# LukasHedegaard/continual-skeletons

Hardware: AMD Instinct MI355X
Metric: clips/sec (ST-GCN clip forward, NTU-60 shape; CoST-GCN online step reported under costgcn_online) (higher is better)
Workload: dtype f32

## Files before the change

### continual-skeletons_amd/blocks.py

```python
import math

import numpy as np
import torch
import torch.nn as nn
from torch.nn.modules.batchnorm import _BatchNorm
from torch.nn.modules.conv import _ConvNd

from . import fold, native


def init_weights(module_, bs=1):
    if isinstance(module_, _ConvNd):
        nn.init.constant_(module_.bias, 0)
        if bs == 1:
            nn.init.kaiming_normal_(module_.weight, mode="fan_out")
        else:
            nn.init.normal_(module_.weight, 0, math.sqrt(2.0 / (module_.weight.numel() * bs)))
    elif isinstance(module_, _BatchNorm):
        nn.init.constant_(module_.weight, bs)
        nn.init.constant_(module_.bias, 0)
    elif isinstance(module_, nn.Linear):
        nn.init.normal_(module_.weight, 0, math.sqrt(2.0 / bs))


# ... 201 lines not shown
        if self.clip_split_k <= 1 or type(self) is not GraphConvolution or self.in_channels < 16:
            return 1
        return max(1, min(self.clip_split_k, -(-self.in_channels // 8)))

    def stage(self, x, y, n_seg, frames, x_strides, y_strides, ksplit=1, partial=None):
        ops = self._packed_ops(x.device)
        if ksplit > 1:
            rc = native.lib().csk_gcn_stage_splitk_f32(
                native.ptr(x), native.ptr(y), native.ptr(ops["w"]), native.ptr(ops["bias"]), native.ptr(ops["ell_src"]),
                native.ptr(ops["ell_val"]), native.ptr(ops["ell_cnt_host"]), ops["ell_w"], n_seg, ops["c_in"], ops["c_out"], frames,
                ops["V"], x_strides[0], x_strides[1], y_strides[0], y_strides[1], ops["res_mode"], ksplit, native.ptr(partial),
                native.stream_of(x))
            native.check(rc, "csk_gcn_stage_splitk_f32")
            return
        gcn_stage(x, y, ops, n_seg=n_seg, frames=frames, x_strides=x_strides, y_strides=y_strides)


def gcn_stage(x, y, ops, n_seg, frames, x_strides, y_strides, adj_seg_stride=0, adj_per_frame=0):
    rc = native.lib().csk_gcn_stage_f32(
        native.ptr(x), native.ptr(y), native.ptr(ops["w"]), native.ptr(ops["bias"]),
        native.ptr(ops["ell_src"]), native.ptr(ops["ell_val"]), native.ptr(ops["ell_cnt_host"]),
        ops["ell_w"], adj_seg_stride, adj_per_frame, n_seg, ops["c_in"], ops["c_out"], frames, ops["V"],
        x_strides[0], x_strides[1], y_strides[0], y_strides[1], ops["res_mode"], native.stream_of(x),
    )
    native.check(rc, "csk_gcn_stage_f32")


class TemporalConvolution(_Folded):

    def __init__(self, in_channels, out_channels, kernel_size=9, stride=1, padding=4):
        super().__init__()
        self.padding = padding
        self.stride = stride
        self.kernel_size = kernel_size
        self.t_conv = nn.Conv2d(in_channels, out_channels, kernel_size=(kernel_size, 1), padding=(padding, 0),
                                stride=(stride, 1))
        self.bn = nn.BatchNorm2d(out_channels)
        init_weights(self.t_conv, bs=1)
        init_weights(self.bn, bs=1)

    def _fold(self):
        f = fold.fold_temporal_conv(self.state_dict())
        f["bias"] = fold.pad_vec(f["bias"])
        return f

    def forward(self, x):
        self._require_eval()
        _check_input(x, self.t_conv.in_channels, "TemporalConvolution input")
        ops = self._packed_ops(x.device)
        return tcn_stage(x, ops["w"], ops["bias"], ops["c_out"], ops["k"], self.stride, self.padding, relu=False)


def tcn_stage(y, w, bias, c_out, k, stride, pad, relu=True, res_mode=0, x_res=None, w_res=None, res_off=0, out=None,
              split=False, ksplit=1, scratch=None, w_wino=None):
    n, c, t_in, v = y.shape
    if t_in + 2 * pad < k:
        raise RuntimeError(f"temporal extent {t_in} (+2*{pad}) shorter than kernel {k}")
    t_out = (t_in + 2 * pad - k) // stride + 1
    if out is None:
        out = torch.empty((n, c_out, t_out, v), device=y.device, dtype=torch.float32)
    elif tuple(out.shape) != (n, c_out, t_out, v) or not out.is_contiguous() or out.dtype != torch.float32 or out.device != y.device:
        raise RuntimeError(f"out must be a contiguous float32 {(n, c_out, t_out, v)} tensor on {y.device}")
    c_res, t_res = (x_res.shape[1], x_res.shape[2]) if x_res is not None else (0, 0)
    if ksplit > 1 and not split:
        if scratch is None:
            raise RuntimeError("tcn_stage: ksplit > 1 needs the owning module's SplitScratch")
        part = scratch.get(y.device, ksplit * n * c_out * t_out * v)
        rc = native.lib().csk_tcn_stage_splitk_f32(
            native.ptr(y), native.ptr(w), native.ptr(x_res), native.ptr(w_res), native.ptr(bias), native.ptr(out),
            n, c, c_out, t_in, v, k, stride, pad, res_mode, c_res, t_res, res_off, int(relu), ksplit, native.ptr(part),
            native.stream_of(y))
        native.check(rc, "csk_tcn_stage_splitk_f32")
        return out
    if w_wino is not None and not split:
        rc = native.lib().csk_tcn_stage_wino_f32(
            native.ptr(y), native.ptr(w), native.ptr(x_res), native.ptr(w_res), native.ptr(bias), native.ptr(out),
            n, c, c_out, t_in, v, k, stride, pad, res_mode, c_res, t_res, res_off, int(relu), native.ptr(w_wino),
            native.stream_of(y))
        native.check(rc, "csk_tcn_stage_wino_f32")
        return out
    fn = native.lib().csk_tcn_stage_bf16x3 if split else native.lib().csk_tcn_stage_f32
    rc = fn(native.ptr(y), native.ptr(w), native.ptr(x_res), native.ptr(w_res), native.ptr(bias), native.ptr(out),
            n, c, c_out, t_in, v, k, stride, pad, res_mode, c_res, t_res, res_off, int(relu), native.stream_of(y))
    native.check(rc, "csk_tcn_stage_bf16x3" if split else "csk_tcn_stage_f32")
    return out


class SpatioTemporalBlock(_Folded):

    def __init__(self, in_channels, out_channels, A, stride=1, residual=True, temporal_kernel_size=9,
                 temporal_padding=-1, GraphConv=GraphConvolution, TempConv=TemporalConvolution):
        super().__init__()
        equal_padding = int((temporal_kernel_size - 1) / 2)
        if temporal_padding < 0:
            temporal_padding = equal_padding
            self.residual_shrink = None
        else:
            assert temporal_padding <= equal_padding
            self.residual_shrink = equal_padding - temporal_padding
        self.stride = stride
        self.gcn = GraphConv(in_channels, out_channels, A)
        self.tcn = TempConv(out_channels, out_channels, stride=stride, kernel_size=temporal_kernel_size,
                            padding=temporal_padding)
        self.relu = nn.ReLU()
        if not residual:
            self.residual = zero
        elif (in_channels == out_channels) and (stride == 1):
            self.residual = unity
        else:
            self.residual = TempConv(in_channels, out_channels, kernel_size=1, stride=stride, padding=0)
        self._native_tail = isinstance(self.tcn, TemporalConvolution) and (
            self.residual in (zero, unity) or isinstance(self.residual, TemporalConvolution)
        )

    precision = "f32"
    clip_split_k = 0
    clip_split_max_seq = CLIP_SPLIT_MAX_SEQUENCES

    def _watched(self):
        return [m for m in (self.tcn, self.residual) if isinstance(m, nn.Module)]

    def _fold(self):
        sd = self.state_dict()
        return fold.fold_block_tail(sd, "", has_conv_residual=isinstance(self.residual, TemporalConvolution),
                                    split=self.precision == "bf16x3", stride=self.stride)

    def forward(self, x, out=None):
        self._require_eval()
        native.require_device_f32(x, "SpatioTemporalBlock input")
        if self._few_channels_fusable(x):
            return self._forward_few_channels(x, out)
        y = self.gcn(x)
        if not self._native_tail:
            z = self.tcn(y)
            r = self.residual(x[:, :, self.residual_shrink:-self.residual_shrink] if self.residual_shrink else x)
            return self.relu(z + r)
        ops = self._packed_ops(x.device)
        shrink = self.residual_shrink or 0
        if self.residual is zero:
            mode, xr = 0, None
        elif self.residual is unity:
            mode, xr = 1, x
        else:
            mode, xr = 2, x
        if self.precision == "bf16x3":
            return tcn_stage(y, ops["w_split"], ops["bias"], ops["c_out"], ops["k"], self.stride, self.tcn.padding, relu=True,
                             res_mode=mode, x_res=xr, w_res=ops["w_res_split"], res_off=shrink, out=out, split=True)
        ks = max(1, min(self.clip_split_k, -(-ops["c"] // 8))) if (self.clip_split_k > 1 and ops["k"] == 9 and y.shape[0] <= self.clip_split_max_seq) else 1
        return tcn_stage(y, ops["w"], ops["bias"], ops["c_out"], ops["k"], self.stride, self.tcn.padding, relu=True,
                         res_mode=mode, x_res=xr, w_res=ops["w_res"], res_off=shrink, out=out, ksplit=ks,
                         scratch=_scratch_of(self) if ks > 1 else None, w_wino=ops["w_wino"] if ks == 1 else None)


def _few_channels_fusable(self, x) -> bool:
    if not self.fuse_few_channels or type(self.gcn) is not GraphConvolution or not self._native_tail:
        return False
    if self.gcn.in_channels > 4 or self.residual is not zero or self.stride != 1 or self.precision != "f32" or self.residual_shrink:
        return False
    if x.dim() != 4 or x.shape[3] not in (18, 25) or self.gcn.precision != "f32":
        return False
    if self.clip_split_k > 1 and x.shape[0] <= self.clip_split_max_seq:
        return False
    g, t = self.gcn._packed_ops(x.device), self._packed_ops(x.device)
    return (t["k"] == 9 and self.tcn.padding == 4 and g["res_mode"] == 2 and g["c_out"] % 8 == 0 and g["V"] == x.shape[3]
            and max(int(v) for v in g["ell_cnt_host"][:2]) <= 1 and int(g["ell_cnt_host"][2]) <= 4)


def _forward_few_channels(self, x, out=None):
    _check_input(x, self.gcn.in_channels, "SpatioTemporalBlock input")
    g, t = self.gcn._packed_ops(x.device), self._packed_ops(x.device)
    n, c, tt, v = x.shape
    if out is None:
        out = torch.empty((n, t["c_out"], tt, v), device=x.device, dtype=torch.float32)
    rc = native.lib().csk_block_few_channels_f32(
        native.ptr(x.contiguous()), native.ptr(g["w"]), native.ptr(g["bias"]), native.ptr(g["ell_src"]), native.ptr(g["ell_val"]),
        native.ptr(g["ell_cnt_host"]), g["ell_w"], native.ptr(t["w"]), native.ptr(t["bias"]), native.ptr(out), n, c, g["c_out"],
        t["c_out"], tt, v, self.tcn.padding, native.stream_of(x))
    native.check(rc, "csk_block_few_channels_f32")
    return out


SpatioTemporalBlock.fuse_few_channels = False
SpatioTemporalBlock._few_channels_fusable = _few_channels_fusable
SpatioTemporalBlock._forward_few_channels = _forward_few_channels


def tcn_step_launch(*args):
    native.check(native.lib().csk_tcn_step_f32(*args), "csk_tcn_step_f32")
```

### continual-skeletons_amd/csrc/tcn_wino.hip

```cpp
#include "mfma_core.h"
#include "tcn_params.h"

namespace {

constexpr int WMT = 64;
constexpr int WNT = 128;
constexpr int WTAPS = 12;

template <int VT>
constexpr int wino_ldb() { return ((2 * ((WNT + VT - 2) / VT) + 10) * VT + 3) / 4 * 4; }

struct WStage12x64 {
    unsigned goff0, loff0, gstride;
    f32x4 v[6];
    __device__ __forceinline__ void setup(int Cpad, int Mpad, int tid) {
        goff0 = (unsigned)(((tid >> 7) * Cpad + ((tid >> 4) & 7)) * Mpad + (tid & 15) * 4);
        loff0 = (unsigned)(tid * 4);
        gstride = (unsigned)(2 * Cpad * Mpad);
    }
    __device__ __forceinline__ void issue_slot(int u, const float *__restrict__ chunk_base) {
        v[u] = *reinterpret_cast<const f32x4 *>(chunk_base + (size_t)u * gstride + goff0);
    }
    __device__ __forceinline__ void issue(const float *__restrict__ chunk_base) {
#pragma unroll
        for (int u = 0; u < 6; ++u) issue_slot(u, chunk_base);
    }
    __device__ __forceinline__ void commit(float *__restrict__ Wl) const {
#pragma unroll
        for (int u = 0; u < 6; ++u) *reinterpret_cast<f32x4 *>(Wl + u * (NTHREADS * 4) + loff0) = v[u];
    }
};

template <int VT, int G>
__device__ __forceinline__ void wino_group(const float *__restrict__ Wl, const float *__restrict__ Bl, int off, int l31, int kh,
                                           f32x16 (&acc)[4][2]) {
    constexpr int LDB = wino_ldb<VT>();
    const float *br = Bl + kh * LDB + off + 3 * G * VT;
    const float *wr = Wl + 4 * G * (KC * WMT) + kh * WMT + l31;
#pragma unroll
    for (int s = 0; s < KC / 2; ++s) {
        const float d0 = br[2 * s * LDB], d1 = br[2 * s * LDB + VT], d2 = br[2 * s * LDB + 2 * VT], d3 = br[2 * s * LDB + 3 * VT];
        const float b[4] = {d0 - d2, d1 + d2, d2 - d1, d1 - d3};
#pragma unroll
        for (int i = 0; i < 4; ++i) {
            const float a0 = wr[i * (KC * WMT) + 2 * s * WMT], a1 = wr[i * (KC * WMT) + 2 * s * WMT + 32];
            acc[i][0] = __builtin_amdgcn_mfma_f32_32x32x2f32(a0, b[i], acc[i][0], 0, 0, 0);
            acc[i][1] = __builtin_amdgcn_mfma_f32_32x32x2f32(a1, b[i], acc[i][1], 0, 0, 0);
        }
    }
}

}

template <int VT>
__global__ __launch_bounds__(NTHREADS, 2) void tcn_stage_wino_kernel(const TcnParams p) {
    constexpr int LDB = wino_ldb<VT>();
    constexpr int NJ = (LDB + 63) / 64;
    extern __shared__ __attribute__((aligned(16))) float smem[];
    float *Wl = smem;
    float *Bl = smem + WTAPS * KC * WMT;

    const int tid = threadIdx.x, lane = tid & 63, wave = __builtin_amdgcn_readfirstlane(tid >> 6);
    const int l31 = lane & 31, kh = lane >> 5;
    const unsigned wid = xcd_contiguous_id(blockIdx.x, gridDim.x);
    const int m0 = (int)(wid % p.mtiles) * WMT, q0 = (int)((wid / p.mtiles) % p.qtiles) * WNT;
    const int seg = (int)(wid / (p.mtiles * p.qtiles));
    const int T = p.Tout, TV = T * VT, QP = p.nt;
    const int qend = min(q0 + WNT, QP);
    const int ja = div_magic(q0, p.vmagic), jb = div_magic(qend - 1, p.vmagic);

    const int qc = min(q0 + wave * 32 + l31, qend - 1);
    const int jc = div_magic(qc, p.vmagic), vc = qc - jc * VT;
    const int off = 2 * (jc - ja) * VT + vc;

    f32x16 acc[4][2];
#pragma unroll
    for (int i = 0; i < 4; ++i)
#pragma unroll
        for (int mi = 0; mi < 2; ++mi)
#pragma unroll
            for (int g = 0; g < 16; ++g) acc[i][mi][g] = 0.f;

    {
        const int fa = 2 * ja - 4;
        const int span = (2 * (jb - ja) + 10) * VT;
        const int64_t cs = (int64_t)TV;
        const float *seg_base = p.y + (int64_t)seg * p.C * cs;
        const float *wbase = p.w + m0;
        WStage12x64 ws;
        ws.setup(p.Cpad, p.Mpad, tid);
        auto kloop = [&](auto &bx) {
            ws.issue(wbase);
            bx.issue(seg_base, p.C, cs, 0, wave);
            for (int c0 = 0; c0 + KC < p.Cpad; c0 += KC) {
                __syncthreads();
                ws.commit(Wl);
                bx.commit(Bl, LDB, wave);
                __syncthreads();
                const float *wnext = wbase + (size_t)(c0 + KC) * p.Mpad;
                const int cn = c0 + KC;
                ws.issue_slot(0, wnext);
                ws.issue_slot(1, wnext);
                bx.template issue_third<0>(seg_base, p.C, cs, cn, wave);
                __builtin_amdgcn_s_setprio(1);
                wino_group<VT, 0>(Wl, Bl, off, l31, kh, acc);
                __builtin_amdgcn_s_setprio(0);
                ws.issue_slot(2, wnext);
                ws.issue_slot(3, wnext);
                bx.template issue_third<1>(seg_base, p.C, cs, cn, wave);
                __builtin_amdgcn_s_setprio(1);
                wino_group<VT, 1>(Wl, Bl, off, l31, kh, acc);
                __builtin_amdgcn_s_setprio(0);
                ws.issue_slot(4, wnext);
                ws.issue_slot(5, wnext);
                bx.template issue_third<2>(seg_base, p.C, cs, cn, wave);
                __builtin_amdgcn_s_setprio(1);
                wino_group<VT, 2>(Wl, Bl, off, l31, kh, acc);
                __builtin_amdgcn_s_setprio(0);
            }
            __syncthreads();
            ws.commit(Wl);
            bx.commit(Bl, LDB, wave);
            __syncthreads();
            wino_group<VT, 0>(Wl, Bl, off, l31, kh, acc);
            wino_group<VT, 1>(Wl, Bl, off, l31, kh, acc);
            wino_group<VT, 2>(Wl, Bl, off, l31, kh, acc);
        };
        const bool interior = fa >= 0 && fa * VT + 4 * ((span + 3) / 4) <= TV;
        if (interior) {
            BStage4<(NJ + 3) / 4> b4;
            b4.setup(fa * VT, span, lane);
            kloop(b4);
        } else {
            BStage<NJ> bs;
            bs.setup(fa * VT, span, TV, lane);
            kloop(bs);
        }
    }

    const bool qv = q0 + wave * 32 + l31 < qend;
    const bool odd_ok = 2 * jc + 1 < T;
    const unsigned p0 = (unsigned)(2 * jc * VT + vc);
    const unsigned b0 = 4u * (4u * (unsigned)kh * (unsigned)TV + p0);
    const unsigned b1 = odd_ok ? b0 + 4u * VT : b0;
    const unsigned kh16 = 16u * (unsigned)kh;
    const float *rseg = p.xres + (int64_t)seg * p.Cout * TV;
    float *oseg = p.out + (int64_t)seg * p.Cout * TV;
#pragma unroll
    for (int mi = 0; mi < 2; ++mi) {
        const int rb = m0 + mi * 32;
        float o0[16], o1[16];
#pragma unroll
        for (int g = 0; g < 16; ++g) {
            const int row = rb + (g & 3) + 8 * (g >> 2);
            const float *rrow = rseg + (int64_t)row * TV;
            const float bias = ld_lane(p.bias + row, kh16);
            const float m1 = acc[1][mi][g], m2 = acc[2][mi][g];
            float v0 = acc[0][mi][g] + m1 + m2 + bias + ld_lane(rrow, b0);
            float v1 = m1 - m2 - acc[3][mi][g] + bias + ld_lane(rrow, b1);
            if (p.relu) { v0 = relu_nan(v0); v1 = relu_nan(v1); }
            o0[g] = v0;
            o1[g] = v1;
        }
        if (qv) {
#pragma unroll
            for (int g = 0; g < 16; ++g) {
                float *orow = oseg + (int64_t)(rb + (g & 3) + 8 * (g >> 2)) * TV;
                st_lane(orow, b0, o0[g]);
                if (odd_ok) st_lane(orow, b1, o1[g]);
            }
        }
    }
}

static int tcn_stage_wino_launch(const float *y, const float *w_wino, const float *x_res, const float *bias, float *out, int n_seg,
                                 int c, int c_out, int t_in, int V, int k, int stride, int pad, int res_mode, int c_res, int t_res,
                                 int res_off, int relu, void *stream) {
    if (!w_wino || !y || !x_res || !bias || !out) return -2;
    if (k != 9 || stride != 1 || pad != 4 || res_mode != CSK_RES_IDENTITY || res_off != 0) return -2;
    if ((V != 25 && V != 18) || c_out % WMT != 0 || c_res != c_out || t_res != t_in || c < 1 || n_seg < 1 || t_in < 1) return -2;
    if ((int64_t)t_in * V >= (1 << 26)) return -2;
    if (csk_diag_flag("CSK_TCN_WINO")) return -2;
    const int qp = (t_in + 1) / 2 * V;
    const int qtiles = (qp + WNT - 1) / WNT, mtiles = c_out / WMT;
    if ((int64_t)qtiles * mtiles * n_seg >= (1ll << 31)) return -2;
    TcnParams p = {};
    p.y = y; p.w = w_wino; p.xres = x_res; p.wres = nullptr; p.bias = bias; p.out = out;
    p.C = c; p.Cpad = round_up(c, CSK_CPAD); p.Cout = c_out; p.Mpad = round_up(c_out, CSK_MT);
    p.Tin = t_in; p.Tout = t_in; p.V = V; p.K = k; p.stride = 1; p.pad = pad;
    p.res_mode = res_mode; p.Cres = c_res; p.CresPad = round_up(c_res, CSK_CPAD); p.Tres = t_res; p.res_off = 0; p.relu = relu;
    p.vmagic = vmagic_of(V); p.mtiles = (unsigned)mtiles; p.qtiles = (unsigned)qtiles; p.nt = qp;
    void (*kern)(TcnParams) = V == 25 ? tcn_stage_wino_kernel<25> : tcn_stage_wino_kernel<18>;
    const int ldb = V == 25 ? wino_ldb<25>() : wino_ldb<18>();
    p.ldb = ldb;
    const size_t lds = (size_t)(WTAPS * KC * WMT + KC * ldb) * sizeof(float);
    if (const int e = csk_ensure_lds((const void *)kern, lds)) return e;
    hipLaunchKernelGGL(kern, dim3((unsigned)(qtiles * mtiles * n_seg)), dim3(NTHREADS), lds, (hipStream_t)stream, p);
    return (int)hipGetLastError();
}

extern "C" int csk_tcn_stage_wino_f32(const float *y, const float *w, const float *x_res, const float *w_res, const float *bias,
                                      float *out, int n_seg, int c, int c_out, int t_in, int V, int k, int stride, int pad,
                                      int res_mode, int c_res, int t_res, int res_off, int relu, const float *w_wino, void *stream) {
    const int rc = tcn_stage_wino_launch(y, w_wino, x_res, bias, out, n_seg, c, c_out, t_in, V, k, stride, pad, res_mode, c_res,
                                         t_res, res_off, relu, stream);
    if (rc != -2) return rc;
    return csk_tcn_stage_f32(y, w, x_res, w_res, bias, out, n_seg, c, c_out, t_in, V, k, stride, pad, res_mode, c_res, t_res,
                             res_off, relu, stream);
}
```

### continual-skeletons_amd/fold.py

```python
from typing import Dict, Optional, Tuple

import numpy as np
import torch

KC = 16
MT = 64
BN_EPS = 1e-5


def _ceil_to(a: int, b: int) -> int:
    return (a + b - 1) // b * b


def bn_affine(weight, bias, mean, var, eps=BN_EPS) -> Tuple[torch.Tensor, torch.Tensor]:
    s = weight.double() / torch.sqrt(var.double() + eps)
    return s, bias.double() - mean.double() * s


def pack_conv_weight(weight: torch.Tensor, scale: torch.Tensor) -> torch.Tensor:
    co, ci, k, _ = weight.shape
    w = weight.double()[:, :, :, 0] * scale[:, None, None]
    out = torch.zeros((k, _ceil_to(ci, KC), _ceil_to(co, MT)), dtype=torch.float64)
    out[:, :ci, :co] = w.permute(2, 1, 0)
    return out.float().contiguous()


WINO_G = ((1.0, 0.0, 0.0), (0.5, 0.5, 0.5), (0.5, -0.5, 0.5), (0.0, 0.0, 1.0))


def pack_conv_weight_wino(weight: torch.Tensor, scale: torch.Tensor) -> torch.Tensor:
    if weight.dim() == 4:
        weight = weight[:, :, :, 0]
    co, ci, k = weight.shape
    if k != 9:
        raise ValueError(f"the Winograd image is built for the 9 x 1 temporal conv, got k = {k}")
    w = weight.double() * scale[:, None, None]
    g = torch.tensor(WINO_G, dtype=torch.float64)
    u = torch.einsum("ir,ocgr->gico", g, w.view(co, ci, 3, 3)).reshape(12, ci, co)
    out = torch.zeros((12, _ceil_to(ci, KC), _ceil_to(co, MT)), dtype=torch.float64)
    out[:, :ci, :co] = u
    return out.float().contiguous()


SPLIT_KS = 16


def split3_bf16(w32: torch.Tensor):
    h = w32.to(torch.bfloat16)
    r1 = w32 - h.float()
    m = r1.to(torch.bfloat16)
    l = (r1 - m.float()).to(torch.bfloat16)
    return h, m, l


def pack_conv_weight_split(weight: torch.Tensor, scale: torch.Tensor, stride: int = 1) -> torch.Tensor:
    if weight.dim() == 4:
        weight = weight[:, :, :, 0]
    co, ci, k = weight.shape
    if k not in (1, 3, 9):
        raise ValueError(f"split weights are built for the 9 x 1 temporal conv, the 1 x 1 residual convs and the 3 graph-conv "
                         f"subsets, got k = {k}")
    w32 = (weight.double() * scale[:, None, None]).float()
    cpad, mpad = _ceil_to(ci, SPLIT_KS), _ceil_to(co, MT)
    taps = [r for rho in range(min(stride, k)) for r in range(rho, k, stride)] if k > 1 else [0]
    slots = _ceil_to(len(taps), 3)
    full = torch.zeros((mpad, cpad, slots), dtype=torch.float32)
    full[:co, :ci, : len(taps)] = w32[:, :, taps]
    pieces = torch.stack([p.view(torch.int16) for p in split3_bf16(full)], 0)
    out = pieces.view(3, mpad, cpad // SPLIT_KS, 2, 8, slots).permute(2, 5, 0, 3, 1, 4)
    return out.contiguous().reshape(-1)


def pad_vec(v: torch.Tensor) -> torch.Tensor:
    out = torch.zeros(_ceil_to(v.numel(), MT), dtype=torch.float64)
    out[: v.numel()] = v
    return out.float().contiguous()


def ell_from_dense(a_eff: torch.Tensor):
    a = a_eff.detach().cpu().double().numpy()
    three, v, _ = a.shape
    nz = a != 0
    per_col = nz.sum(axis=1)
    cnt = per_col.max(axis=1).astype(np.int32)
    ew = max(1, int(cnt.max()))
    src = np.zeros((three, v, ew), dtype=np.int32)
    val = np.zeros((three, v, ew), dtype=np.float32)
    for i in range(three):
        for w in range(v):
            rows = np.nonzero(nz[i, :, w])[0]
            src[i, w, : len(rows)] = rows
            val[i, w, : len(rows)] = a[i, rows, w]
    return torch.from_numpy(src), torch.from_numpy(val), torch.from_numpy(cnt), ew


def fold_graph_conv(sd: Dict[str, torch.Tensor], p: str = "", split: bool = False) -> dict:
    sd = {k: v.detach().cpu() for k, v in sd.items() if k.startswith(p)}
    s, t = bn_affine(sd[p + "bn.weight"], sd[p + "bn.bias"], sd[p + "bn.running_mean"], sd[p + "bn.running_var"])
    co, ci = sd[p + "g_conv.0.weight"].shape[:2]
    conv_res = (p + "gcn_residual.0.weight") in sd
    r = 4 if conv_res else 3
    w = torch.zeros((r, _ceil_to(ci, KC), _ceil_to(co, MT)), dtype=torch.float64)
    bias = t.clone()
    for i in range(3):
        w[i, :ci, :co] = (sd[f"{p}g_conv.{i}.weight"].double()[:, :, 0, 0] * s[:, None]).t()
        bias += s * sd[f"{p}g_conv.{i}.bias"].double()
    if conv_res:
        sr, tr = bn_affine(sd[p + "gcn_residual.1.weight"], sd[p + "gcn_residual.1.bias"],
                           sd[p + "gcn_residual.1.running_mean"], sd[p + "gcn_residual.1.running_var"])
        w[3, :ci, :co] = (sd[p + "gcn_residual.0.weight"].double()[:, :, 0, 0] * sr[:, None]).t()
        bias += sr * sd[p + "gcn_residual.0.bias"].double() + tr
    a_eff = sd[p + "A"].double() * sd[p + "graph_attn"].double()
    src, val, cnt, ew = ell_from_dense(a_eff)
    out = dict(w=w.float().contiguous(), bias=pad_vec(bias), ell_src=src, ell_val=val, ell_cnt_host=cnt,
               ell_w=ew, c_in=ci, c_out=co, res_mode=2 if conv_res else 1, V=a_eff.shape[-1], w_split=None, w_res_split=None)
    if split:
        one = torch.ones(co, dtype=torch.float64)
        w3 = w[:3, :ci, :co].permute(2, 1, 0).contiguous()
        out["w_split"] = pack_conv_weight_split(w3, one)
        if conv_res:
            out["w_res_split"] = pack_conv_weight_split(w[3, :ci, :co].t().contiguous().unsqueeze(-1), one)
    return out


def fold_temporal_conv(sd: Dict[str, torch.Tensor], p: str = "", wino: bool = False) -> dict:
    s, t = bn_affine(sd[p + "bn.weight"].cpu(), sd[p + "bn.bias"].cpu(), sd[p + "bn.running_mean"].cpu(),
                     sd[p + "bn.running_var"].cpu())
    wt = sd[p + "t_conv.weight"].detach().cpu()
    bias = s * sd[p + "t_conv.bias"].detach().cpu().double() + t
    w_wino = pack_conv_weight_wino(wt, s) if wino and wt.shape[2] == 9 else None
    return dict(w=pack_conv_weight(wt, s), bias=bias, c_in=wt.shape[1], c_out=wt.shape[0], k=wt.shape[2], w_wino=w_wino)


def fold_temporal_conv_split(sd: Dict[str, torch.Tensor], p: str = "", stride: int = 1) -> torch.Tensor:
    s, _ = bn_affine(sd[p + "bn.weight"].cpu(), sd[p + "bn.bias"].cpu(), sd[p + "bn.running_mean"].cpu(),
                     sd[p + "bn.running_var"].cpu())
    return pack_conv_weight_split(sd[p + "t_conv.weight"].detach().cpu(), s, stride)


def fold_block_tail(sd: Dict[str, torch.Tensor], p: str = "", has_conv_residual: Optional[bool] = None,
                    split: bool = False, stride: int = 1) -> dict:
    main = fold_temporal_conv(sd, p + "tcn.", wino=stride == 1)
    out = dict(w=main["w"], k=main["k"], c=main["c_in"], c_out=main["c_out"], w_res=None, c_res=0, w_split=None, w_res_split=None,
               w_wino=main["w_wino"])
    bias = main["bias"]
    if has_conv_residual is None:
        has_conv_residual = (p + "residual.t_conv.weight") in sd
    if has_conv_residual:
        res = fold_temporal_conv(sd, p + "residual.")
        out["w_res"], out["c_res"] = res["w"], res["c_in"]
        bias = bias + res["bias"]
    if split:
        out["w_split"] = fold_temporal_conv_split(sd, p + "tcn.", stride)
        if has_conv_residual:
            out["w_res_split"] = fold_temporal_conv_split(sd, p + "residual.")
    out["bias"] = pad_vec(bias)
    return out


def fold_data_bn(sd: Dict[str, torch.Tensor], p: str = "data_bn."):
    s, t = bn_affine(sd[p + "weight"].cpu(), sd[p + "bias"].cpu(), sd[p + "running_mean"].cpu(),
                     sd[p + "running_var"].cpu())
    return s.float().contiguous(), t.float().contiguous()
```

### continual-skeletons_amd/native.py

```python
import ctypes as C
import os

import torch

_HERE = os.path.dirname(os.path.abspath(__file__))
LIB_PATH = os.path.join(_HERE, "libcskel_hip.so")
ABI_VERSION = 16

_p, _i, _l = C.c_void_p, C.c_int, C.c_int64
SIGNATURES = {
    "csk_abi_version": [],
    "csk_stream_overlap_probe": [C.c_void_p, C.c_void_p, C.c_int, C.POINTER(C.c_float)],
    "csk_gcn_stage_f32": [_p, _p, _p, _p, _p, _p, _p, _i, _l, _i, _i, _i, _i, _i, _i, _l, _l, _l, _l, _i, _p],
    "csk_gcn_stage_splitk_f32": [_p, _p, _p, _p, _p, _p, _p, _i, _i, _i, _i, _i, _i, _l, _l, _l, _l, _i, _i, _p, _p],
    "csk_tcn_stage_f32": [_p, _p, _p, _p, _p, _p, _i, _i, _i, _i, _i, _i, _i, _i, _i, _i, _i, _i, _i, _p],
    "csk_tcn_stage_wino_f32": [_p, _p, _p, _p, _p, _p, _i, _i, _i, _i, _i, _i, _i, _i, _i, _i, _i, _i, _i, _p, _p],
    "csk_block_few_channels_f32": [_p, _p, _p, _p, _p, _p, _i, _p, _p, _p, _i, _i, _i, _i, _i, _i, _i, _p],
    "csk_tcn_stage_splitk_f32": [_p, _p, _p, _p, _p, _p, _i, _i, _i, _i, _i, _i, _i, _i, _i, _i, _i, _i, _i, _i, _p, _p],
    "csk_conv1x1_f32": [_p, _p, _p, _p, _i, _i, _i, _i, _i, _l, _l, _l, _l, _p],
    "csk_tcn_stage_bf16x3": [_p, _p, _p, _p, _p, _p, _i, _i, _i, _i, _i, _i, _i, _i, _i, _i, _i, _i, _i, _p],
    "csk_gcn_stage_bf16x3": [_p, _p, _p, _p, _p, _p, _p, _p, _i, _i, _i, _i, _i, _i, _i, _p],
    "csk_input_norm_f32": [_p, _p, _p, _p, _i, _i, _i, _i, _i, _l, _l, _p],
    "csk_pool_fc_f32": [_p, _p, _p, _p, _p, _i, _i, _i, _i, _i, _p],
    "csk_fc_f32": [_p, _p, _p, _p, _i, _i, _i, _p],
    "csk_pool_scaled_f32": [_p, _p, _i, _i, _i, _i, C.c_float, _p],
    "csk_agcn_attention_f32": [_p, _p, _p, _p, _i, _i, _i, _i, _l, _l, _i, _l, _p],
    "csk_agcn_embed_attention_f32": [_p, _p, _p, _p, _p, _p, _i, _i, _i, _i, _i, _i, _l, _l, _p],
    "csk_tcn_step_f32": [_p, _i, _i, _i, _i, _p, _p, _i, _i, _i, _p, _p, _p, _i, _i, _i, _i, _l, _i, _i, _i, _i, _i, _p, _p],
    "csk_co_stack_step_f32": [_i, _p, _i, _i, _l, _p],
    "csk_co_block_step_f32": [_p, _i, _i, _i, _p, _p, _p, _p, _p, _i, _i, _p, _i, _i, _p, _p, _i, _i, _p, _i, _i, _i, _i, _i, _l, _p],
    "csk_co_spatial_pool_f32": [_p, _p, _i, _i, _i, _l, _p],
    "csk_co_window_mean_f32": [_p, _p, _l, _i, _i, _i, _p],
    "csk_co_head_step_f32": [_p, _p, _p, _p, _p, _p, _i, _i, _i, _l, _i, _i, _i, _i, _i, _p],
    "csk_input_norm_frames_f32": [_p, _p, _i, _p, _p, _i, _i, _i, _i, _l, _p],

    "csk_fuse_rank_f32": [_p, _i, _i, _i, _i, _l, _l, _p, _p, _p, _p],
    "csk_co_plan_create": [_i, _p, _p, _i, _i, _i, _i, _i, _l, _p, _p, _i, _p, _p, _i, _i, _p, _p],
    "csk_co_plan_destroy": [_p],
    "csk_co_plan_update_weights": [_p, _i, _p, _p, _p, _p, _p],
    "csk_co_plan_set_fusion": [_p, _i],
    "csk_co_plan_cycle": [_p, C.POINTER(C.c_int64), _i, _p, _i, _p, _p, _p, _p, _p],
    "csk_str_unit_f32": [_p, _p, _p, _l, _p, _p, _p, _p, _p, _p, _p, _i, _i, _i, _i, _i, _l, _l, _l, _l, _p],
}
RESTYPES = {"csk_co_plan_create": C.c_void_p, "csk_co_plan_destroy": None}


class CoLayer(C.Structure):
    _fields_ = [("c_in", C.c_int32), ("c_out", C.c_int32), ("stride", C.c_int32), ("res_kind", C.c_int32),
                ("gcn_res_mode", C.c_int32), ("ell_w", C.c_int32), ("ell_cnt", C.c_int32 * 3), ("tcn_ksplit", C.c_int32),
                ("y_slots", C.c_int32), ("out_slots", C.c_int32), ("partial_emits", C.c_int32), ("agcn_adj_frames", C.c_int32),
                ("gcn_ksplit", C.c_int32), ("gcn_partial_frames", C.c_int32),
                ("gcn_w", C.c_void_p), ("gcn_bias", C.c_void_p), ("ell_src", C.c_void_p), ("ell_val", C.c_void_p),
                ("tcn_w", C.c_void_p), ("tcn_w_res", C.c_void_p), ("tcn_bias", C.c_void_p),
                ("y_ring", C.c_void_p), ("out_ring", C.c_void_p), ("tcn_partial", C.c_void_p),
                ("agcn_inter", C.c_int32), ("agcn_pad_", C.c_int32), ("agcn_w_pairs", C.c_void_p), ("agcn_b_pairs", C.c_void_p),
                ("agcn_a_sum", C.c_void_p), ("agcn_adj", C.c_void_p)]


_lib = None


def lib():
    global _lib
    if _lib is None:
        if not os.path.exists(LIB_PATH):
            raise RuntimeError(
                f"{LIB_PATH} not found: the HIP library is not built. "
                "Run `python -c 'import __graft_entry__ as g; g.build()'` (needs hipcc); there is no CPU fallback."
            )
# ... 42 lines not shown
```

### include/cskel.h

```cpp
#ifndef CSKEL_H
#define CSKEL_H

#include <stdint.h>

#ifdef __cplusplus
extern "C" {
#endif

#define CSK_ABI_VERSION 16
#define CSK_KC 8
#define CSK_CPAD 16
#define CSK_MT 64

#define CSK_RES_NONE 0
#define CSK_RES_IDENTITY 1
#define CSK_RES_CONV 2

int csk_abi_version(void);
const char *csk_last_error(void);

int csk_stream_overlap_probe(void *stream_a, void *stream_b, int spin_us, float *ratio);

int csk_gcn_stage_f32(const float *x, float *y, const float *w, const float *bias,
                      const int32_t *ell_src, const float *ell_val, const int32_t *ell_cnt,
                      int ell_w, int64_t adj_seg_stride, int adj_per_frame,
                      int n_seg, int c_in, int c_out, int frames, int V,
                      int64_t x_seg_stride, int64_t x_chan_stride,
                      int64_t y_seg_stride, int64_t y_chan_stride,
                      int res_mode, void *stream);

int csk_gcn_stage_splitk_f32(const float *x, float *y, const float *w, const float *bias, const int32_t *ell_src,
                             const float *ell_val, const int32_t *ell_cnt, int ell_w, int n_seg, int c_in, int c_out,
                             int frames, int V, int64_t x_seg_stride, int64_t x_chan_stride, int64_t y_seg_stride,
                             int64_t y_chan_stride, int res_mode, int ksplit, float *partial, void *stream);

int csk_tcn_stage_f32(const float *y, const float *w, const float *x_res, const float *w_res,
                      const float *bias, float *out,
                      int n_seg, int c, int c_out, int t_in, int V, int k, int stride, int pad,
                      int res_mode, int c_res, int t_res, int res_off, int relu, void *stream);

int csk_tcn_stage_wino_f32(const float *y, const float *w, const float *x_res, const float *w_res,
                           const float *bias, float *out,
                           int n_seg, int c, int c_out, int t_in, int V, int k, int stride, int pad,
                           int res_mode, int c_res, int t_res, int res_off, int relu, const float *w_wino, void *stream);

int csk_block_few_channels_f32(const float *x, const float *gcn_w, const float *gcn_bias, const int32_t *ell_src,
                               const float *ell_val, const int32_t *ell_cnt, int ell_w, const float *tcn_w,
                               const float *tcn_bias, float *out, int n_seg, int c_in, int c_mid, int c_out, int t_in,
                               int V, int pad, void *stream);

int csk_tcn_stage_splitk_f32(const float *y, const float *w, const float *x_res, const float *w_res,
                             const float *bias, float *out,
                             int n_seg, int c, int c_out, int t_in, int V, int k, int stride, int pad,
                             int res_mode, int c_res, int t_res, int res_off, int relu, int ksplit, float *partial,
                             void *stream);

int csk_conv1x1_f32(const float *x, float *y, const float *w, const float *bias, int n_seg, int c_in, int c_out,
                    int frames, int V, int64_t x_seg_stride, int64_t x_chan_stride, int64_t y_seg_stride,
                    int64_t y_chan_stride, void *stream);

int csk_tcn_stage_bf16x3(const float *y, const void *w_split, const float *x_res, const void *w_res_split,
                         const float *bias, float *out,
                         int n_seg, int c, int c_out, int t_in, int V, int k, int stride, int pad,
                         int res_mode, int c_res, int t_res, int res_off, int relu, void *stream);

int csk_gcn_stage_bf16x3(const float *x, float *y, const void *w_split, const void *w_res_split, const float *bias,
                         const int32_t *ell_src, const float *ell_val, const int32_t *ell_cnt, int ell_w,
                         int n_seg, int c_in, int c_out, int frames, int V, int res_mode, void *stream);

int csk_input_norm_f32(const float *x, const float *scale, const float *shift, float *h,
                       int N, int C, int T, int V, int M,
                       int64_t h_seg_stride, int64_t h_chan_stride, void *stream);

int csk_pool_fc_f32(const float *h, const float *fc_w, const float *fc_b, float *feat, float *logits,
                    int N, int M, int C, int TV, int classes, void *stream);

int csk_pool_scaled_f32(const float *h, float *feat, int N, int M, int C, int TV, float scale, void *stream);

int csk_fc_f32(const float *feat, const float *fc_w, const float *fc_b, float *logits,
               int N, int C, int classes, void *stream);

int csk_agcn_attention_f32(const float *E, const float *a_sum, float *ell_val, float *scratch, int n_seg, int inter, int T,
                           int V, int64_t e_seg_stride, int64_t e_chan_stride, int seg_per_group, int64_t e_group_stride,
                           void *stream);

int csk_agcn_embed_attention_f32(const float *x, const float *w_pairs, const float *b_pairs, const float *a_sum, float *ell_val,
                                 float *scratch, int n_seg, int c_in, int inter, int frames, int V, int per_frame,
                                 int64_t x_seg_stride, int64_t x_chan_stride, void *stream);


int csk_tcn_step_f32(const float *ring, int slots, int head, int head_step, int n_emit, const float *w,
                     const float *x_res, int x_res_slots, int x_res_slot0, int x_res_step,
                     const float *w_res, const float *bias, float *out, int out_slots, int out_slot0,
                     int c, int c_out, int64_t P, int k, int res_mode, int c_res, int relu, int ksplit, float *partial,
                     void *stream);

int csk_co_block_step_f32(const float *xin, int xin_slots, int xin_slot0, int c_in, const float *gcn_w,
// ... 84 lines not shown
```

Baseline: 4073.

## Add stride-2 Winograd temporal conv kernel and extend Winograd to no-residual blocks

```diff
diff --git a/continual-skeletons_amd/blocks.py b/continual-skeletons_amd/blocks.py
--- a/continual-skeletons_amd/blocks.py
+++ b/continual-skeletons_amd/blocks.py
@@ -277,7 +277,7 @@
 
 
 def tcn_stage(y, w, bias, c_out, k, stride, pad, relu=True, res_mode=0, x_res=None, w_res=None, res_off=0, out=None,
-              split=False, ksplit=1, scratch=None, w_wino=None):
+              split=False, ksplit=1, scratch=None, w_wino=None, w_wino2=None):
     n, c, t_in, v = y.shape
     if t_in + 2 * pad < k:
         raise RuntimeError(f"temporal extent {t_in} (+2*{pad}) shorter than kernel {k}")
@@ -296,6 +296,13 @@
             n, c, c_out, t_in, v, k, stride, pad, res_mode, c_res, t_res, res_off, int(relu), ksplit, native.ptr(part),
             native.stream_of(y))
         native.check(rc, "csk_tcn_stage_splitk_f32")
+        return out
+    if w_wino2 is not None and not split:
+        rc = native.lib().csk_tcn_stage_wino2_f32(
+            native.ptr(y), native.ptr(w), native.ptr(x_res), native.ptr(w_res), native.ptr(bias), native.ptr(out),
+            n, c, c_out, t_in, v, k, stride, pad, res_mode, c_res, t_res, res_off, int(relu), native.ptr(w_wino2),
+            native.stream_of(y))
+        native.check(rc, "csk_tcn_stage_wino2_f32")
         return out
     if w_wino is not None and not split:
         rc = native.lib().csk_tcn_stage_wino_f32(
@@ -372,9 +379,15 @@
             return tcn_stage(y, ops["w_split"], ops["bias"], ops["c_out"], ops["k"], self.stride, self.tcn.padding, relu=True,
                              res_mode=mode, x_res=xr, w_res=ops["w_res_split"], res_off=shrink, out=out, split=True)
         ks = max(1, min(self.clip_split_k, -(-ops["c"] // 8))) if (self.clip_split_k > 1 and ops["k"] == 9 and y.shape[0] <= self.clip_split_max_seq) else 1
+        w2 = None
+        if ks == 1 and not shrink and not self._few_channel_first_block():
+            w2 = ops["w_wino_s2"] if self.stride == 2 else ops["w_wino"] if mode == 0 else None
         return tcn_stage(y, ops["w"], ops["bias"], ops["c_out"], ops["k"], self.stride, self.tcn.padding, relu=True,
                          res_mode=mode, x_res=xr, w_res=ops["w_res"], res_off=shrink, out=out, ksplit=ks,
-                         scratch=_scratch_of(self) if ks > 1 else None, w_wino=ops["w_wino"] if ks == 1 else None)
+                         scratch=_scratch_of(self) if ks > 1 else None, w_wino=ops["w_wino"] if ks == 1 else None, w_wino2=w2)
+
+    def _few_channel_first_block(self) -> bool:
+        return type(self.gcn) is GraphConvolution and self.gcn.in_channels <= 4 and self.residual is zero
 
 
 def _few_channels_fusable(self, x) -> bool:
diff --git a/continual-skeletons_amd/csrc/tcn_wino.hip b/continual-skeletons_amd/csrc/tcn_wino.hip
--- a/continual-skeletons_amd/csrc/tcn_wino.hip
+++ b/continual-skeletons_amd/csrc/tcn_wino.hip
@@ -52,7 +52,7 @@
 
 }
 
-template <int VT>
+template <int VT, bool RES>
 __global__ __launch_bounds__(NTHREADS, 2) void tcn_stage_wino_kernel(const TcnParams p) {
     constexpr int LDB = wino_ldb<VT>();
     constexpr int NJ = (LDB + 63) / 64;
@@ -156,8 +156,12 @@
             const float *rrow = rseg + (int64_t)row * TV;
             const float bias = ld_lane(p.bias + row, kh16);
             const float m1 = acc[1][mi][g], m2 = acc[2][mi][g];
-            float v0 = acc[0][mi][g] + m1 + m2 + bias + ld_lane(rrow, b0);
-            float v1 = m1 - m2 - acc[3][mi][g] + bias + ld_lane(rrow, b1);
+            float v0 = acc[0][mi][g] + m1 + m2 + bias;
+            float v1 = m1 - m2 - acc[3][mi][g] + bias;
+            if (RES) {
+                v0 += ld_lane(rrow, b0);
+                v1 += ld_lane(rrow, b1);
+            }
             if (p.relu) { v0 = relu_nan(v0); v1 = relu_nan(v1); }
             o0[g] = v0;
             o1[g] = v1;
@@ -173,24 +177,250 @@
     }
 }
 
+namespace {
+
+constexpr int W2TAPS = 13;
+
+struct Wino2Group { int s0, w0, points; };
+constexpr Wino2Group WINO2_GROUPS[4] = {{0, 0, 4}, {6, 4, 3}, {1, 7, 3}, {5, 10, 3}};
+
+template <int VT>
+constexpr int wino2_ldb() { return ((4 * ((WNT + VT - 2) / VT) + 11) * VT + 3) / 4 * 4; }
+
+struct WStage13x64 {
+    unsigned goff0, loff0, gstride, u6;
+    f32x4 v[7];
+    __device__ __forceinline__ void setup(int Cpad, int Mpad, int tid) {
+        goff0 = (unsigned)(((tid >> 7) * Cpad + ((tid >> 4) & 7)) * Mpad + (tid & 15) * 4);
+        loff0 = (unsigned)(tid * 4);
+        gstride = (unsigned)(2 * Cpad * Mpad);
+        u6 = tid >= 128 ? 5u : 6u;
+    }
+    __device__ __forceinline__ void issue_slot(int u, const float *__restrict__ chunk_base) {
+        if (u < 6) v[u] = *reinterpret_cast<const f32x4 *>(chunk_base + (size_t)u * gstride + goff0);
+        else v[6] = *reinterpret_cast<const f32x4 *>(chunk_base + (size_t)u6 * gstride + goff0);
+    }
+    __device__ __forceinline__ void issue(const float *__restrict__ chunk_base) {
+#pragma unroll
+        for (int u = 0; u < 7; ++u) issue_slot(u, chunk_base);
+    }
+    __device__ __forceinline__ void commit(float *__restrict__ Wl) const {
+#pragma unroll
+        for (int u = 0; u < 6; ++u) *reinterpret_cast<f32x4 *>(Wl + u * (NTHREADS * 4) + loff0) = v[u];
+        *reinterpret_cast<f32x4 *>(Wl + u6 * (NTHREADS * 4) + loff0) = v[6];
+    }
+};
+
+template <int VT, int G>
+__device__ __forceinline__ void wino2_group(const float *__restrict__ Wl, const float *__restrict__ Bl, int off, int l31, int kh,
+                                            f32x16 (&acc)[4][2]) {
+    constexpr int LDB = wino2_ldb<VT>();
+    constexpr Wino2Group grp = WINO2_GROUPS[G];
+    const float *br = Bl + kh * LDB + off + grp.s0 * VT;
+    const float *wr = Wl + grp.w0 * (KC * WMT) + kh * WMT + l31;
+#pragma unroll
+    for (int s = 0; s < KC / 2; ++s) {
+        const float d0 = br[2 * s * LDB], d1 = br[2 * s * LDB + 2 * VT], d2 = br[2 * s * LDB + 4 * VT];
+        float b[4] = {d0 - d2, d1 + d2, d2 - d1, 0.f};
+        if (grp.points == 4) b[3] = d1 - br[2 * s * LDB + 6 * VT];
+#pragma unroll
+        for (int i = 0; i < grp.points; ++i) {
+            const float a0 = wr[i * (KC * WMT) + 2 * s * WMT], a1 = wr[i * (KC * WMT) + 2 * s * WMT + 32];
+            acc[i][0] = __builtin_amdgcn_mfma_f32_32x32x2f32(a0, b[i], acc[i][0], 0, 0, 0);
+            acc[i][1] = __builtin_amdgcn_mfma_f32_32x32x2f32(a1, b[i], acc[i][1], 0, 0, 0);
+        }
+    }
+}
+
+template <int VT>
+__device__ __forceinline__ void wino2_residual(const float *__restrict__ Wl, const float *__restrict__ Bl, int off, int l31, int kh,
+                                               f32x16 (&acc)[4][2]) {
+    constexpr int LDB = wino2_ldb<VT>();
+    const float *br = Bl + kh * LDB + off + 4 * VT;
+    const float *wr = Wl + kh * WMT + l31;
+#pragma unroll
+    for (int s = 0; s < KC / 2; ++s) {
+        const float x0 = br[2 * s * LDB], x1 = -br[2 * s * LDB + 2 * VT];
+        const float a0 = wr[2 * s * WMT], a1 = wr[2 * s * WMT + 32];
+        acc[0][0] = __builtin_amdgcn_mfma_f32_32x32x2f32(a0, x0, acc[0][0], 0, 0, 0);
+        acc[0][1] = __builtin_amdgcn_mfma_f32_32x32x2f32(a1, x0, acc[0][1], 0, 0, 0);
+        acc[3][0] = __builtin_amdgcn_mfma_f32_32x32x2f32(a0, x1, acc[3][0], 0, 0, 0);
+        acc[3][1] = __builtin_amdgcn_mfma_f32_32x32x2f32(a1, x1, acc[3][1], 0, 0, 0);
+    }
+}
+
+}
+
+template <int VT, bool RESCONV>
+__global__ __launch_bounds__(NTHREADS, 2) void tcn_stage_wino2_kernel(const TcnParams p) {
+    constexpr int LDB = wino2_ldb<VT>();
+    constexpr int NJ = (LDB + 63) / 64;
+    extern __shared__ __attribute__((aligned(16))) float smem[];
+    float *Wl = smem;
+    float *Bl = smem + W2TAPS * KC * WMT;
+
+    const int tid = threadIdx.x, lane = tid & 63, wave = __builtin_amdgcn_readfirstlane(tid >> 6);
+    const int l31 = lane & 31, kh = lane >> 5;
+    const unsigned wid = xcd_contiguous_id(blockIdx.x, gridDim.x);
+    const int m0 = (int)(wid % p.mtiles) * WMT, q0 = (int)((wid / p.mtiles) % p.qtiles) * WNT;
+    const int seg = (int)(wid / (p.mtiles * p.qtiles));
+    const int TVi = p.Tin * VT, TVo = p.Tout * VT, QP = p.nt;
+    const int qend = min(q0 + WNT, QP);
+    const int ja = div_magic(q0, p.vmagic), jb = div_magic(qend - 1, p.vmagic);
+
+    const int qc = min(q0 + wave * 32 + l31, qend - 1);
+    const int jc = div_magic(qc, p.vmagic), vc = qc - jc * VT;
+    const int off = 4 * (jc - ja) * VT + vc;
+
+    f32x16 acc[4][2];
+#pragma unroll
+    for (int i = 0; i < 4; ++i)
+#pragma unroll
+        for (int mi = 0; mi < 2; ++mi)
+#pragma unroll
+            for (int g = 0; g < 16; ++g) acc[i][mi][g] = 0.f;
+
+    {
+        const int fa = 4 * ja - 4;
+        const int span = (4 * (jb - ja) + 11) * VT;
+        const int64_t cs = (int64_t)TVi;
+        const float *seg_base = p.y + (int64_t)seg * p.C * cs;
+        const float *rseg_base = p.xres + (int64_t)seg * p.Cres * cs;
+        const float *wbase = p.w + m0;
+        const float *rwbase = p.wres + m0 + ((tid >> 4) & 7) * p.Mpad + (tid & 15) * 4;
+        float *rwl = Wl + (tid & 127) * 4;
+        WStage13x64 ws;
+        ws.setup(p.Cpad, p.Mpad, tid);
+        auto groups = [&]() {
+            wino2_group<VT, 0>(Wl, Bl, off, l31, kh, acc);
+            wino2_group<VT, 1>(Wl, Bl, off, l31, kh, acc);
+            wino2_group<VT, 2>(Wl, Bl, off, l31, kh, acc);
+            wino2_group<VT, 3>(Wl, Bl, off, l31, kh, acc);
+        };
+        auto kloop = [&](auto &bx) {
+            ws.issue(wbase);
+            bx.issue(seg_base, p.C, cs, 0, wave);
+            for (int c0 = 0; c0 + KC < p.Cpad; c0 += KC) {
+                __syncthreads();
+                ws.commit(Wl);
+                bx.commit(Bl, LDB, wave);
+                __syncthreads();
+                const float *wnext = wbase + (size_t)(c0 + KC) * p.Mpad;
+                const int cn = c0 + KC;
+                ws.issue_slot(0, wnext);
+                ws.issue_slot(1, wnext);
+                bx.template issue_third<0>(seg_base, p.C, cs, cn, wave);
+                __builtin_amdgcn_s_setprio(1);
+                wino2_group<VT, 0>(Wl, Bl, off, l31, kh, acc);
+                __builtin_amdgcn_s_setprio(0);
+                ws.issue_slot(2, wnext);
+                ws.issue_slot(3, wnext);
+                bx.template issue_third<1>(seg_base, p.C, cs, cn, wave);
+                __builtin_amdgcn_s_setprio(1);
+                wino2_group<VT, 1>(Wl, Bl, off, l31, kh, acc);
+                __builtin_amdgcn_s_setprio(0);
+                ws.issue_slot(4, wnext);
+                ws.issue_slot(5, wnext);
+                bx.template issue_third<2>(seg_base, p.C, cs, cn, wave);
+                __builtin_amdgcn_s_setprio(1);
+                wino2_group<VT, 2>(Wl, Bl, off, l31, kh, acc);
+                __builtin_amdgcn_s_setprio(0);
+                ws.issue_slot(6, wnext);
+                __builtin_amdgcn_s_setprio(1);
+                wino2_group<VT, 3>(Wl, Bl, off, l31, kh, acc);
+                __builtin_amdgcn_s_setprio(0);
+            }
+            __syncthreads();
+            ws.commit(Wl);
+            bx.commit(Bl, LDB, wave);
+            __syncthreads();
+            if (!RESCONV) {
+                groups();
+                return;
+            }
+            f32x4 rw = *reinterpret_cast<const f32x4 *>(rwbase);
+            bx.issue(rseg_base, p.Cres, cs, 0, wave);
+            groups();
+            for (int c0 = 0; c0 + KC < p.CresPad; c0 += KC) {
+                __syncthreads();
+                *reinterpret_cast<f32x4 *>(rwl) = rw;
+                bx.commit(Bl, LDB, wave);
+                __syncthreads();
+                rw = *reinterpret_cast<const f32x4 *>(rwbase + (size_t)(c0 + KC) * p.Mpad);
+                bx.issue(rseg_base, p.Cres, cs, c0 + KC, wave);
+                wino2_residual<VT>(Wl, Bl, off, l31, kh, acc);
+            }
+            __syncthreads();
+            *reinterpret_cast<f32x4 *>(rwl) = rw;
+            bx.commit(Bl, LDB, wave);
+            __syncthreads();
+            wino2_residual<VT>(Wl, Bl, off, l31, kh, acc);
+        };
+        const bool interior = fa >= 0 && fa * VT + 4 * ((span + 3) / 4) <= TVi;
+        if (interior) {
+            BStage4<(NJ + 3) / 4> b4;
+            b4.setup(fa * VT, span, lane);
+            kloop(b4);
+        } else {
+            BStage<NJ> bs;
+            bs.setup(fa * VT, span, TVi, lane);
+            kloop(bs);
+        }
+    }
+
+    const bool qv = q0 + wave * 32 + l31 < qend;
+    const bool odd_ok = 2 * jc + 1 < p.Tout;
+    const unsigned p0 = (unsigned)(2 * jc * VT + vc);
+    const unsigned b0 = 4u * (4u * (unsigned)kh * (unsigned)TVo + p0);
+    const unsigned b1 = b0 + 4u * VT;
+    const unsigned kh16 = 16u * (unsigned)kh;
+    float *oseg = p.out + (int64_t)seg * p.Cout * TVo;
+#pragma unroll
+    for (int mi = 0; mi < 2; ++mi) {
+        const int rb = m0 + mi * 32;
+        float o0[16], o1[16];
+#pragma unroll
+        for (int g = 0; g < 16; ++g) {
+            const float bias = ld_lane(p.bias + rb + (g & 3) + 8 * (g >> 2), kh16);
+            const float m1 = acc[1][mi][g], m2 = acc[2][mi][g];
+            float v0 = acc[0][mi][g] + m1 + m2 + bias;
+            float v1 = m1 - m2 - acc[3][mi][g] + bias;
+            if (p.relu) { v0 = relu_nan(v0); v1 = relu_nan(v1); }
+            o0[g] = v0;
+            o1[g] = v1;
+        }
+        if (qv) {
+#pragma unroll
+            for (int g = 0; g < 16; ++g) {
+                float *orow = oseg + (int64_t)(rb + (g & 3) + 8 * (g >> 2)) * TVo;
+                st_lane(orow, b0, o0[g]);
+                if (odd_ok) st_lane(orow, b1, o1[g]);
+            }
+        }
+    }
+}
+
 static int tcn_stage_wino_launch(const float *y, const float *w_wino, const float *x_res, const float *bias, float *out, int n_seg,
                                  int c, int c_out, int t_in, int V, int k, int stride, int pad, int res_mode, int c_res, int t_res,
-                                 int res_off, int relu, void *stream) {
-    if (!w_wino || !y || !x_res || !bias || !out) return -2;
-    if (k != 9 || stride != 1 || pad != 4 || res_mode != CSK_RES_IDENTITY || res_off != 0) return -2;
-    if ((V != 25 && V != 18) || c_out % WMT != 0 || c_res != c_out || t_res != t_in || c < 1 || n_seg < 1 || t_in < 1) return -2;
+                                 int res_off, int relu, bool allow_none, void *stream) {
+    const bool none = allow_none && res_mode == CSK_RES_NONE;
+    if (!w_wino || !y || !bias || !out) return -2;
+    if (k != 9 || stride != 1 || pad != 4 || res_off != 0) return -2;
+    if (!none && (res_mode != CSK_RES_IDENTITY || !x_res || c_res != c_out || t_res != t_in)) return -2;
+    if ((V != 25 && V != 18) || c_out % WMT != 0 || c < 1 || n_seg < 1 || t_in < 1) return -2;
     if ((int64_t)t_in * V >= (1 << 26)) return -2;
     if (csk_diag_flag("CSK_TCN_WINO")) return -2;
     const int qp = (t_in + 1) / 2 * V;
     const int qtiles = (qp + WNT - 1) / WNT, mtiles = c_out / WMT;
     if ((int64_t)qtiles * mtiles * n_seg >= (1ll << 31)) return -2;
     TcnParams p = {};
-    p.y = y; p.w = w_wino; p.xres = x_res; p.wres = nullptr; p.bias = bias; p.out = out;
+    p.y = y; p.w = w_wino; p.xres = none ? y : x_res; p.wres = nullptr; p.bias = bias; p.out = out;
     p.C = c; p.Cpad = round_up(c, CSK_CPAD); p.Cout = c_out; p.Mpad = round_up(c_out, CSK_MT);
     p.Tin = t_in; p.Tout = t_in; p.V = V; p.K = k; p.stride = 1; p.pad = pad;
-    p.res_mode = res_mode; p.Cres = c_res; p.CresPad = round_up(c_res, CSK_CPAD); p.Tres = t_res; p.res_off = 0; p.relu = relu;
+    p.res_mode = res_mode; p.Cres = c_out; p.CresPad = round_up(c_out, CSK_CPAD); p.Tres = t_in; p.res_off = 0; p.relu = relu;
     p.vmagic = vmagic_of(V); p.mtiles = (unsigned)mtiles; p.qtiles = (unsigned)qtiles; p.nt = qp;
-    void (*kern)(TcnParams) = V == 25 ? tcn_stage_wino_kernel<25> : tcn_stage_wino_kernel<18>;
+    void (*kern)(TcnParams) = V == 25 ? (none ? tcn_stage_wino_kernel<25, false> : tcn_stage_wino_kernel<25, true>)
+                                      : (none ? tcn_stage_wino_kernel<18, false> : tcn_stage_wino_kernel<18, true>);
     const int ldb = V == 25 ? wino_ldb<25>() : wino_ldb<18>();
     p.ldb = ldb;
     const size_t lds = (size_t)(WTAPS * KC * WMT + KC * ldb) * sizeof(float);
@@ -199,12 +429,57 @@
     return (int)hipGetLastError();
 }
 
+static int tcn_stage_wino2_launch(const float *y, const float *w_wino2, const float *x_res, const float *w_res, const float *bias,
+                                  float *out, int n_seg, int c, int c_out, int t_in, int V, int k, int stride, int pad, int res_mode,
+                                  int c_res, int t_res, int res_off, int relu, void *stream) {
+    if (!w_wino2 || !y || !bias || !out) return -2;
+    if (k != 9 || stride != 2 || pad != 4 || res_off != 0) return -2;
+    const bool conv = res_mode == CSK_RES_CONV;
+    if (!conv && res_mode != CSK_RES_NONE) return -2;
+    if (conv && (!x_res || !w_res || c_res < 1 || t_res != t_in)) return -2;
+    if ((V != 25 && V != 18) || c_out % WMT != 0 || c < 1 || n_seg < 1 || t_in < 1) return -2;
+    if ((int64_t)t_in * V >= (1 << 26)) return -2;
+    if (csk_diag_flag("CSK_TCN_WINO")) return -2;
+    const int t_out = (t_in - 1) / 2 + 1;
+    const int qp = (t_out + 1) / 2 * V;
+    const int qtiles = (qp + WNT - 1) / WNT, mtiles = c_out / WMT;
+    if ((int64_t)qtiles * mtiles * n_seg >= (1ll << 31)) return -2;
+    TcnParams p = {};
+    p.y = y; p.w = w_wino2; p.xres = conv ? x_res : y; p.wres = conv ? w_res : w_wino2; p.bias = bias; p.out = out;
+    p.C = c; p.Cpad = round_up(c, CSK_CPAD); p.Cout = c_out; p.Mpad = round_up(c_out, CSK_MT);
+    p.Tin = t_in; p.Tout = t_out; p.V = V; p.K = k; p.stride = 2; p.pad = pad;
+    p.res_mode = res_mode; p.Cres = conv ? c_res : 1; p.CresPad = round_up(p.Cres, CSK_CPAD); p.Tres = t_in; p.res_off = 0;
+    p.relu = relu;
+    p.vmagic = vmagic_of(V); p.mtiles = (unsigned)mtiles; p.qtiles = (unsigned)qtiles; p.nt = qp;
+    void (*kern)(TcnParams) = V == 25 ? (conv ? tcn_stage_wino2_kernel<25, true> : tcn_stage_wino2_kernel<25, false>)
+                                      : (conv ? tcn_stage_wino2_kernel<18, true> : tcn_stage_wino2_kernel<18, false>);
+    const int ldb = V == 25 ? wino2_ldb<25>() : wino2_ldb<18>();
+    p.ldb = ldb;
+    const size_t lds = (size_t)(W2TAPS * KC * WMT + KC * ldb) * sizeof(float);
+    if (const int e = csk_ensure_lds((const void *)kern, lds)) return e;
+    hipLaunchKernelGGL(kern, dim3((unsigned)(qtiles * mtiles * n_seg)), dim3(NTHREADS), lds, (hipStream_t)stream, p);
+    return (int)hipGetLastError();
+}
+
 extern "C" int csk_tcn_stage_wino_f32(const float *y, const float *w, const float *x_res, const float *w_res, const float *bias,
                                       float *out, int n_seg, int c, int c_out, int t_in, int V, int k, int stride, int pad,
                                       int res_mode, int c_res, int t_res, int res_off, int relu, const float *w_wino, void *stream) {
     const int rc = tcn_stage_wino_launch(y, w_wino, x_res, bias, out, n_seg, c, c_out, t_in, V, k, stride, pad, res_mode, c_res,
-                                         t_res, res_off, relu, stream);
+                                         t_res, res_off, relu, false, stream);
     if (rc != -2) return rc;
     return csk_tcn_stage_f32(y, w, x_res, w_res, bias, out, n_seg, c, c_out, t_in, V, k, stride, pad, res_mode, c_res, t_res,
                              res_off, relu, stream);
 }
+
+extern "C" int csk_tcn_stage_wino2_f32(const float *y, const float *w, const float *x_res, const float *w_res, const float *bias,
+                                       float *out, int n_seg, int c, int c_out, int t_in, int V, int k, int stride, int pad,
+                                       int res_mode, int c_res, int t_res, int res_off, int relu, const float *w_wino,
+                                       void *stream) {
+    const int rc = stride == 2 ? tcn_stage_wino2_launch(y, w_wino, x_res, w_res, bias, out, n_seg, c, c_out, t_in, V, k, stride, pad,
+                                                        res_mode, c_res, t_res, res_off, relu, stream)
+                               : tcn_stage_wino_launch(y, w_wino, x_res, bias, out, n_seg, c, c_out, t_in, V, k, stride, pad,
+                                                       res_mode, c_res, t_res, res_off, relu, true, stream);
+    if (rc != -2) return rc;
+    return csk_tcn_stage_f32(y, w, x_res, w_res, bias, out, n_seg, c, c_out, t_in, V, k, stride, pad, res_mode, c_res, t_res,
+                             res_off, relu, stream);
+}
diff --git a/continual-skeletons_amd/fold.py b/continual-skeletons_amd/fold.py
--- a/continual-skeletons_amd/fold.py
+++ b/continual-skeletons_amd/fold.py
@@ -38,6 +38,28 @@
     g = torch.tensor(WINO_G, dtype=torch.float64)
     u = torch.einsum("ir,ocgr->gico", g, w.view(co, ci, 3, 3)).reshape(12, ci, co)
     out = torch.zeros((12, _ceil_to(ci, KC), _ceil_to(co, MT)), dtype=torch.float64)
+    out[:, :ci, :co] = u
+    return out.float().contiguous()
+
+
+WINO_S2_GROUPS = ((0, 2, 4), (6, 8, None), (1, 3, None), (5, 7, None))
+
+
+def pack_conv_weight_wino_s2(weight: torch.Tensor, scale: torch.Tensor) -> torch.Tensor:
+    if weight.dim() == 4:
+        weight = weight[:, :, :, 0]
+    co, ci, k = weight.shape
+    if k != 9:
+        raise ValueError(f"the Winograd image is built for the 9 x 1 temporal conv, got k = {k}")
+    w = weight.double() * scale[:, None, None]
+    g = torch.tensor(WINO_G, dtype=torch.float64)
+    slots = []
+    for taps in WINO_S2_GROUPS:
+        grp = torch.stack([w[:, :, r] if r is not None else torch.zeros_like(w[:, :, 0]) for r in taps], -1)
+        u = torch.einsum("ir,ocr->ico", g, grp)
+        slots.append(u if taps[2] is not None else u[:3])
+    u = torch.cat(slots, 0)
+    out = torch.zeros((13, _ceil_to(ci, KC), _ceil_to(co, MT)), dtype=torch.float64)
     out[:, :ci, :co] = u
     return out.float().contiguous()
 
@@ -123,13 +145,15 @@
     return out
 
 
-def fold_temporal_conv(sd: Dict[str, torch.Tensor], p: str = "", wino: bool = False) -> dict:
+def fold_temporal_conv(sd: Dict[str, torch.Tensor], p: str = "", wino: bool = False, wino_s2: bool = False) -> dict:
     s, t = bn_affine(sd[p + "bn.weight"].cpu(), sd[p + "bn.bias"].cpu(), sd[p + "bn.running_mean"].cpu(),
                      sd[p + "bn.running_var"].cpu())
     wt = sd[p + "t_conv.weight"].detach().cpu()
     bias = s * sd[p + "t_conv.bias"].detach().cpu().double() + t
     w_wino = pack_conv_weight_wino(wt, s) if wino and wt.shape[2] == 9 else None
-    return dict(w=pack_conv_weight(wt, s), bias=bias, c_in=wt.shape[1], c_out=wt.shape[0], k=wt.shape[2], w_wino=w_wino)
+    w_wino_s2 = pack_conv_weight_wino_s2(wt, s) if wino_s2 and wt.shape[2] == 9 else None
+    return dict(w=pack_conv_weight(wt, s), bias=bias, c_in=wt.shape[1], c_out=wt.shape[0], k=wt.shape[2], w_wino=w_wino,
+                w_wino_s2=w_wino_s2)
 
 
 def fold_temporal_conv_split(sd: Dict[str, torch.Tensor], p: str = "", stride: int = 1) -> torch.Tensor:
@@ -140,9 +164,9 @@
 
 def fold_block_tail(sd: Dict[str, torch.Tensor], p: str = "", has_conv_residual: Optional[bool] = None,
                     split: bool = False, stride: int = 1) -> dict:
-    main = fold_temporal_conv(sd, p + "tcn.", wino=stride == 1)
+    main = fold_temporal_conv(sd, p + "tcn.", wino=stride == 1, wino_s2=stride == 2)
     out = dict(w=main["w"], k=main["k"], c=main["c_in"], c_out=main["c_out"], w_res=None, c_res=0, w_split=None, w_res_split=None,
-               w_wino=main["w_wino"])
+               w_wino=main["w_wino"], w_wino_s2=main["w_wino_s2"])
     bias = main["bias"]
     if has_conv_residual is None:
         has_conv_residual = (p + "residual.t_conv.weight") in sd
diff --git a/continual-skeletons_amd/native.py b/continual-skeletons_amd/native.py
--- a/continual-skeletons_amd/native.py
+++ b/continual-skeletons_amd/native.py
@@ -15,6 +15,7 @@
     "csk_gcn_stage_splitk_f32": [_p, _p, _p, _p, _p, _p, _p, _i, _i, _i, _i, _i, _i, _l, _l, _l, _l, _i, _i, _p, _p],
     "csk_tcn_stage_f32": [_p, _p, _p, _p, _p, _p, _i, _i, _i, _i, _i, _i, _i, _i, _i, _i, _i, _i, _i, _p],
     "csk_tcn_stage_wino_f32": [_p, _p, _p, _p, _p, _p, _i, _i, _i, _i, _i, _i, _i, _i, _i, _i, _i, _i, _i, _p, _p],
+    "csk_tcn_stage_wino2_f32": [_p, _p, _p, _p, _p, _p, _i, _i, _i, _i, _i, _i, _i, _i, _i, _i, _i, _i, _i, _p, _p],
     "csk_block_few_channels_f32": [_p, _p, _p, _p, _p, _p, _i, _p, _p, _p, _i, _i, _i, _i, _i, _i, _i, _p],
     "csk_tcn_stage_splitk_f32": [_p, _p, _p, _p, _p, _p, _i, _i, _i, _i, _i, _i, _i, _i, _i, _i, _i, _i, _i, _i, _p, _p],
     "csk_conv1x1_f32": [_p, _p, _p, _p, _i, _i, _i, _i, _i, _l, _l, _l, _l, _p],
diff --git a/include/cskel.h b/include/cskel.h
--- a/include/cskel.h
+++ b/include/cskel.h
@@ -43,6 +43,11 @@
                            const float *bias, float *out,
                            int n_seg, int c, int c_out, int t_in, int V, int k, int stride, int pad,
                            int res_mode, int c_res, int t_res, int res_off, int relu, const float *w_wino, void *stream);
+
+int csk_tcn_stage_wino2_f32(const float *y, const float *w, const float *x_res, const float *w_res,
+                            const float *bias, float *out,
+                            int n_seg, int c, int c_out, int t_in, int V, int k, int stride, int pad,
+                            int res_mode, int c_res, int t_res, int res_off, int relu, const float *w_wino, void *stream);
 
 int csk_block_few_channels_f32(const float *x, const float *gcn_w, const float *gcn_bias, const int32_t *ell_src,
                                const float *ell_val, const int32_t *ell_cnt, int ell_w, const float *tcn_w,
```

Result: faster. 4189, median of 6 (+2.9%).
